# leohuang2013/pyannote-audio_speaker-diarization_cpp

Hardware: AMD Instinct MI355X
Metric: real-time factor (audio-sec/wall-sec), 1 h 16 kHz mono per GPU (higher is better)
Workload: dtype f32

## Files before the change

pyannote-audio_speaker-diarization_cpp_amd/csrc/api.cpp:

```cpp
#include "common.h"
#include <algorithm>
#include <cmath>
#include <cstdlib>

static std::string g_create_err;

int seg_prec(const sd_ctx* c) { return c->seg_precision >= 0 ? c->seg_precision : (c->ecapa_precision != 0 ? 3 : 0); }

extern "C" const char* sd_create_error(void) { return g_create_err.c_str(); }
extern "C" const char* sd_last_error(const sd_ctx* c) { return c ? c->err.c_str() : "null context"; }

extern "C" sd_ctx* sd_create(const char* seg_path, const char* emb_path, int device)
{
    g_create_err.clear();
    int ndev = 0;
    if (hipGetDeviceCount(&ndev) != hipSuccess || ndev <= 0) { g_create_err = "no HIP device available (libsdhip has no CPU fallback)"; return nullptr; }
    if (device < 0 || device >= ndev) { g_create_err = "device id out of range"; return nullptr; }
    if (hipSetDevice(device) != hipSuccess) { g_create_err = "hipSetDevice failed"; return nullptr; }
    sd_ctx* c = new sd_ctx();
    c->device = device;
    hipDeviceProp_t prop;
    if (hipGetDeviceProperties(&prop, device) == hipSuccess) c->num_cu = prop.multiProcessorCount;
    if (hipStreamCreateWithFlags(&c->stream, hipStreamNonBlocking) != hipSuccess) { g_create_err = "hipStreamCreate failed"; delete c; return nullptr; }
    auto fail = [&](const std::string& m) { g_create_err = m; sd_destroy(c); return (sd_ctx*)nullptr; };
// ... 28 lines not shown
    while (!c->streams.empty()) sd_stream_close(c->streams.back());
    for (void* p : c->owned) (void)hipFree(p);
    for (auto& kv : c->ws) kv.second.release();
    if (c->stream) (void)hipStreamDestroy(c->stream);
    delete c;
}

void sd_flush_profile(sd_ctx* c)
{
    for (auto& t : c->pending) {
        hipEvent_t e0 = std::get<1>(t), e1 = std::get<2>(t);
        float ms = 0;
        if (hipEventSynchronize(e1) == hipSuccess) (void)hipEventElapsedTime(&ms, e0, e1);
        KernelStat& s = c->stats[std::get<0>(t)];
        s.ms += ms; s.launches++; s.flops += std::get<3>(t); s.bytes += std::get<4>(t);
        (void)hipEventDestroy(e0); (void)hipEventDestroy(e1);
    }
    c->pending.clear();
}

extern "C" int sd_kernel_stats(const sd_ctx* cc, const char* kernel, double* total_ms, int64_t* launches, double* flops, double* bytes)
{
    sd_ctx* c = const_cast<sd_ctx*>(cc);
    if (!c || !kernel) return SD_ERR_ARG;
    (void)hipStreamSynchronize(c->stream);
    sd_flush_profile(c);
    auto it = c->stats.find(kernel);
    KernelStat s; if (it != c->stats.end()) s = it->second;
    if (total_ms) *total_ms = s.ms; if (launches) *launches = s.launches; if (flops) *flops = s.flops; if (bytes) *bytes = s.bytes;
    return SD_OK;
}
extern "C" int sd_debug_read_ws(sd_ctx* c, const char* name, int64_t offset, void* h_out, int64_t bytes)
{
    if (!c || !name || !h_out || offset < 0 || bytes < 0) return SD_ERR_ARG;
    auto it = c->ws.find(name);
    if (it == c->ws.end() || !it->second.p) SD_FAIL(c, SD_ERR_ARG, "no workspace named %s", name);
    if ((size_t)(offset + bytes) > it->second.cap) SD_FAIL(c, SD_ERR_ARG, "workspace %s holds %zu bytes", name, it->second.cap);
    HIPCHK(c, hipStreamSynchronize(c->stream));
    HIPCHK(c, hipMemcpy(h_out, (const char*)it->second.p + offset, (size_t)bytes, hipMemcpyDeviceToHost));
    return SD_OK;
}
extern "C" void sd_reset_stats(sd_ctx* c) { if (!c) return; (void)hipStreamSynchronize(c->stream); sd_flush_profile(c); c->stats.clear(); }
extern "C" int sd_stage_ms(const sd_ctx* c, double* ms4) { if (!c || !ms4) return SD_ERR_ARG; for (int i = 0; i < 4; ++i) ms4[i] = c->stage_ms[i]; return SD_OK; }
extern "C" int sd_set_option(sd_ctx* c, const char* key, int64_t v)
{
    if (!c || !key) return SD_ERR_ARG;
    std::string k(key);
    if (k == "emb_batch_items") { c->emb_batch_items = v; c->emb_batch_explicit = true; }
    else if (k == "seg_batch_chunks") c->seg_batch_chunks = v;
    else if (k == "ws_limit_mb") g_ws_limit.store(v > 0 ? (size_t)v << 20 : 0);
    else if (k == "emb_batch_default") { c->emb_batch_items = 3072; c->emb_batch_explicit = false; c->embed_calls = v; }
    else if (k == "linkage_wgs") c->linkage_wgs = v;
    else if (k == "linkage_threads") c->linkage_threads = v;
    else if (k == "linkage_kernel") c->linkage_kernel = v;
    else if (k == "linkage_tie_kernel") c->linkage_tie_kernel = v;
    else if (k == "linkage_zero_phase") c->linkage_zero_phase = v;
    else if (k == "linkage_force_heap") c->linkage_force_heap = v != 0;
    else if (k == "linkage_hx_wide") c->linkage_hx_wide = v != 0;
    else if (k == "linkage_prefetch") c->linkage_prefetch = v != 0;
    else if (k == "linkage_one_xcd") c->linkage_one_xcd = v;
    else if (k == "linkage_square") c->linkage_square = v;
    else if (k == "skip_dead_rows") c->skip_dead_rows = v != 0;
    else if (k == "conv_h256") c->conv_h256 = v != 0;
    else if (k == "conv_glds") c->conv_glds = v != 0;
    else if (k == "conv_pp") c->conv_pp = v != 0;
    else if (k == "conv_glds_f32") c->conv_glds_f32 = v != 0;
    else if (k == "conv_mfma16") { if (v < 0 || v > 2) return SD_ERR_ARG; c->conv_mfma16 = (int)v; }
    else if (k == "conv_rot") { if (v < 0 || v > 3) return SD_ERR_ARG; c->conv_rot = (int)v; }
    else if (k == "conv_stagger") { if (v < 0 || v > 2) return SD_ERR_ARG; c->conv_stagger = (int)v; }
    else if (k == "conv_w256_f32") c->conv_w256_f32 = v != 0;
    else if (k == "conv_pn") c->conv_pn = (int)v;
    else if (k == "ecapa_ld_pad") { if (v < 0 || v > 1024 || ((int64_t)v & 7)) return SD_ERR_ARG; c->ecapa_ld_pad = (int)v; }
    else if (k == "seg_shared_conv0") c->seg_shared_conv0 = v != 0;
    else if (k == "seg_wide_ih") c->seg_wide_ih = v != 0;
    else if (k == "conv_w256_kmin") c->conv_w256_kmin = (int)v;
    else if (k == "conv_pn128") c->conv_pn128 = (int)v;
    else if (k == "seg_precision") { if (v != 0 && v != 3 && v != -1) SD_FAIL(c, SD_ERR_ARG, "seg_precision must be 0 (f32), 3 (split fp16 operands for the LSTM) or -1 (auto: 3 whenever ecapa_precision is not 0)"); c->seg_precision = (int)v; }
    else if (k == "ecapa_precision") { if (v < 0 || v > 3) SD_FAIL(c, SD_ERR_ARG, "ecapa_precision must be 0 (f32), 1 (fp16), 2 (fp16, hi + lo weight planes) or 3 (f32 tensors, split fp16 operands on the wide layers)");
                                        if (hipSetDevice(c->device) != hipSuccess) SD_FAIL(c, SD_ERR_HIP, "hipSetDevice failed");
                                        const int rcw = ensure_ecapa_mode_weights(c, (int)v); if (rcw) return rcw;
                                        c->ecapa_precision = (int)v; }
    else if (k == "ecapa_f16_hp") { if (v != 0 && v != 1 && v != 3) SD_FAIL(c, SD_ERR_ARG, "ecapa_f16_hp must be 0, 1 (MFA output in f32) or 3 (+ the attention branch)"); c->ecapa_f16_hp = (int)v; }
    else if (k == "ecapa_keep_cat") c->ecapa_keep_cat = v != 0;
    else if (k == "rank0_permille") c->rank0_permille = (int)v;
    else if (k == "virtual_world") c->virtual_world = (int)v;
    else if (k == "comm_timeout_ms") c->comm_timeout_ms = v;
    else if (k == "inject_fail_rank") c->inject_fail_rank = (int)v;
    else if (k == "constrained_assignment") c->constrained_assignment = v != 0;
    else if (k == "clustering_method") { if (v < SD_LINKAGE_SINGLE || v > SD_LINKAGE_WEIGHTED) SD_FAIL(c, SD_ERR_ARG, "clustering_method must be one of SD_LINKAGE_SINGLE (0) .. SD_LINKAGE_WEIGHTED (6)"); c->clustering_method = (int)v; }
    else if (k == "min_cluster_size") { if (v < 1 || v > 0x7fffffff) SD_FAIL(c, SD_ERR_ARG, "min_cluster_size must be at least 1"); c->min_cluster_size = (int)v; }
    else if (k == "num_clusters") c->num_clusters = (int)v;
    else if (k == "min_clusters") c->min_clusters = (int)v;
    else if (k == "max_clusters") c->max_clusters = (int)v;
    else if (k == "activity_hamming") { if (v != 0 && v != 1) SD_FAIL(c, SD_ERR_ARG, "activity_hamming must be 0 or 1"); c->activity_hamming = v != 0; }
    else if (k == "profile") { c->profile = v != 0; c->profile_detail = v >= 2; }
    else SD_FAIL(c, SD_ERR_ARG, "unknown option %s", key);
    return SD_OK;
}

extern "C" int sd_set_option_f64(sd_ctx* c, const char* key, double v)
{
    if (!c || !key) return SD_ERR_ARG;
    std::string k(key);
    if (k == "clustering_threshold") { if (!(v >= 0.0 && v <= 2.0)) SD_FAIL(c, SD_ERR_ARG, "clustering_threshold must lie in [0, 2]"); c->clustering_threshold = v; }
    else if (k == "activity_onset") { if (!(v >= 0.0 && v <= 1.0)) SD_FAIL(c, SD_ERR_ARG, "activity_onset must lie in [0, 1]"); c->activity_onset = v; }
    else if (k == "activity_offset") { if (!(v >= 0.0 && v <= 1.0)) SD_FAIL(c, SD_ERR_ARG, "activity_offset must lie in [0, 1]"); c->activity_offset = v; }
    else if (k == "activity_min_duration_on") { if (!(v >= 0.0)) SD_FAIL(c, SD_ERR_ARG, "activity_min_duration_on must be >= 0"); c->activity_min_on = v; }
    else if (k == "activity_min_duration_off") { if (!(v >= 0.0)) SD_FAIL(c, SD_ERR_ARG, "activity_min_duration_off must be >= 0"); c->activity_min_off = v; }
    else SD_FAIL(c, SD_ERR_ARG, "unknown real-valued option %s", key);
    return SD_OK;
}
extern "C" int sd_linkage_method_from_name(const char* name)
{
    static const char* const names[] = {"single", "complete", "average", "centroid", "median", "ward", "weighted"};
    if (!name) return -1;
    for (int i = 0; i < 7; ++i) if (std::string(name) == names[i]) return i;
    return -1;
}

extern "C" int64_t sd_num_chunks(int64_t n, int64_t* last_len)
{
    int64_t i = 0, cnt = 0;
    if (n > SD_CHUNK) { cnt = (n - SD_CHUNK + SD_HOP - 1) / SD_HOP; i = cnt * SD_HOP; }
    int64_t ll = 0;
    if (i + 1 < n) { ll = n - i; cnt++; }
    if (last_len) *last_len = ll;
    return cnt;
}

extern "C" int sd_embed_dev(sd_ctx* c, const float* d_wav, int64_t n, const float* d_masks, int64_t items, int64_t first_item, float* d_emb)
{
    ENTER(c);
    if (!d_wav || !d_masks || !d_emb || n <= 0 || items < 0) SD_FAIL(c, SD_ERR_ARG, "sd_embed_dev: bad argument");
    int rc = run_embed(c, d_wav, n, d_masks, items, first_item, d_emb);
    if (rc) return rc;
    HIPCHK(c, hipStreamSynchronize(c->stream));
    return SD_OK;
}

extern "C" int sd_embed(sd_ctx* c, const float* h_wav, int64_t n, const float* h_masks, int64_t items, float* h_emb)
{
    ENTER(c);
    if (!h_wav || !h_masks || !h_emb || n <= 0 || items < 0) SD_FAIL(c, SD_ERR_ARG, "sd_embed: bad argument");
    DTMP(c, dw, n * sizeof(float)); DTMP(c, dm, items * SD_FRAMES * sizeof(float)); DTMP(c, de, items * SD_EMB_DIM * sizeof(float));
    HIPCHK(c, hipMemcpy(dw.p, h_wav, n * sizeof(float), hipMemcpyHostToDevice));
    HIPCHK(c, hipMemcpy(dm.p, h_masks, items * SD_FRAMES * sizeof(float), hipMemcpyHostToDevice));
    int rc = run_embed(c, (const float*)dw.p, n, (const float*)dm.p, items, 0, (float*)de.p);
    if (rc) return rc;
    HIPCHK(c, hipStreamSynchronize(c->stream));
    HIPCHK(c, hipMemcpy(h_emb, de.p, items * SD_EMB_DIM * sizeof(float), hipMemcpyDeviceToHost));
    return SD_OK;
}

extern "C" int sd_frontend(sd_ctx* c, const float* h_wav, int64_t n, const float* h_masks, int64_t items, float* h_feats, float* h_lens)
{
    ENTER(c);
    if (!h_wav || !h_masks || n <= 0 || items <= 0) SD_FAIL(c, SD_ERR_ARG, "sd_frontend: bad argument");
    DTMP(c, dw, n * sizeof(float)); DTMP(c, dm, items * SD_FRAMES * sizeof(float));
    DTMP(c, df, items * SD_TP * SD_FEAT_LD * sizeof(float)); DTMP(c, dl, items * sizeof(float));
    DTMP(c, dn, items * sizeof(int)); DTMP(c, dv, items * sizeof(int)); DTMP(c, dg, items * sizeof(int)); DTMP(c, dr, (items + 1) * sizeof(int));
    HIPCHK(c, hipMemcpy(dw.p, h_wav, n * sizeof(float), hipMemcpyHostToDevice));
    HIPCHK(c, hipMemcpy(dm.p, h_masks, items * SD_FRAMES * sizeof(float), hipMemcpyHostToDevice));
    std::vector<int> ro((size_t)items + 1);
    for (int64_t i = 0; i <= items; ++i) ro[(size_t)i] = (int)(i * SD_TP);
    HIPCHK(c, hipMemcpy(dr.p, ro.data(), ro.size() * sizeof(int), hipMemcpyHostToDevice));
    int rc = frontend_prepare(c, (const float*)dm.p, items, 0, (float*)dl.p, (int*)dn.p, (int*)dv.p, (int*)dg.p, false, nullptr, nullptr);
// ... 238 lines not shown
```

pyannote-audio_speaker-diarization_cpp_amd/csrc/common.h:

```cpp
#pragma once
#include <hip/hip_runtime.h>
#include <atomic>
#include <chrono>
#include <cstdint>
#include <cstdio>
#include <cstring>
#include <map>
#include <set>
#include <string>
#include <functional>
#include <initializer_list>
#include <vector>
#include "../../include/sdhip_test.h"

#define SD_T 501
#define SD_TP 501
#define SD_NBINS 201
#define SD_NMELS 80
#define SD_FEAT_LD 96

struct KernelStat { double ms = 0; int64_t launches = 0; double flops = 0, bytes = 0; };

inline std::atomic<long long> g_ws_alloc_us{0}, g_ws_free_us{0};
inline std::atomic<size_t> g_ws_alloc_bytes{0}, g_ws_allocs{0};
// ... 42 lines not shown
    int TpIn, TpOut;
    int Tin, T;
    int Cin, Cout, KT, dil;
    int cin_real;
    int pad_mode;
    int act1, act2;
    int m_tiles, n_tiles;
    int sched;
    const int2* rowtab;
    int in_rows;
    int y_f32;
    int kt_real;
    int prec;
    const void* W16x;
    float acc_scale;
    int stagger;
};
#define ROWTAB_T(y) ((y) & 1023)
#define ROWTAB_LAST(y) (((y) >> 10) & 1023)
#define ROWTAB_ITEM(y) ((int)((unsigned)(y) >> 20))
#define ROWTAB_MAX_ITEMS 4095
#define SD_SKINNY_MAX_ROWS 4096

struct EcapaWeights {
    bool loaded = false;
    float* mel_w = nullptr; int* mel_lo = nullptr; int* mel_cnt = nullptr; int* mel_off = nullptr; int mel_nnz = 0;
    float* window = nullptr;
    double* tw_cos = nullptr;
    double* tw_nsin = nullptr;
    ConvLayer block0;
    struct SERes { ConvLayer tdnn1, res[7], tdnn2, se1, se2; int dil; } blk[3];
    ConvLayer mfa, asp_tdnn_x, asp_tdnn_ms, asp_conv, fc;
    int C = 1024;
    std::vector<ConvLayer*> conv16;
    bool have16 = false, have16x = false;
};

struct SegWeights {
    bool loaded = false;
    float wn_w = 1, wn_b = 0;
    ConvLayer conv0, conv1, conv2;
    float* conv0_wsum = nullptr;
    float* in_w[3] = {nullptr, nullptr, nullptr};
    float* in_b[3] = {nullptr, nullptr, nullptr};
    ConvLayer lstm_ih[4];
    float* lstm_hh[4][2] = {};
    void* lstm_hh_x[4][2] = {};
    float lstm_hh_inv[4][2] = {};
    ConvLayer lin0, lin1;
    float* cls_w = nullptr; float* cls_b = nullptr;
};

struct StepStash {
    bool clustered = false;
    int64_t N = 0; int K = 0;
    std::vector<int> clusters, cluster_res, hard_pre;
    std::vector<double> X, Xn, soft;
    int64_t ar0 = 0, cr0 = 0, rows = 0, crow_all = 0, nact = 0;
    int64_t infer_items = 0;
};

struct sd_ctx {
    int device = 0;
    hipStream_t stream = nullptr;
    std::string err;
    EcapaWeights ew;
    SegWeights sw;
    std::vector<void*> owned;
    char* warena_cur = nullptr; size_t warena_left = 0;
    std::map<std::string, DevBuf> ws;
    std::set<std::string> rs_taps_filled;
    std::map<std::string, KernelStat> stats;
    bool profile = false;
    bool profile_detail = false;
    std::vector<std::tuple<std::string, hipEvent_t, hipEvent_t, double, double>> pending;
    double stage_ms[4] = {0, 0, 0, 0};
    int64_t emb_batch_items = 3072;
    bool emb_batch_explicit = false;
    int64_t embed_calls = 0;
    int64_t seg_batch_chunks = 4096;
    int num_clusters = -1, min_clusters = -1, max_clusters = -1;
    int ecapa_precision = 0;
    int seg_precision = -1;
    bool ecapa_keep_cat = false;
    int ecapa_f16_hp = 0;
    bool conv_w256_f32 = true;
    int conv_pn128 = 0;
    int ecapa_ld_pad = 0;
    bool wav_padded = false;
    bool seg_wide_ih = true;
    bool seg_shared_conv0 = true;
    int conv_w256_kmin = 0;
    int conv_pn = 0;
    bool conv_h256 = true;
    int conv_mfma16 = 1;
    int conv_rot = 3;
    int conv_stagger = 0;
    bool conv_glds_f32 = false;
    bool conv_pp = true;
    bool conv_glds = true;
    bool skip_dead_rows = true;
    int64_t linkage_wgs = -1;
    int64_t linkage_square = -1;
    int64_t linkage_one_xcd = 1;
    int64_t linkage_zero_phase = 1;
    int64_t linkage_tie_kernel = 1;
    int64_t linkage_prefetch = 0;
    bool linkage_hx_wide = false;
    bool linkage_force_heap = false;
    int64_t linkage_kernel = -1;
    int64_t linkage_threads = 0;
    int num_cu = 256;
    bool constrained_assignment = false;
    int clustering_method = SD_LINKAGE_CENTROID;
    double clustering_threshold = (double)0.7153814381597874f;
    int min_cluster_size = 15;
    std::vector<double> last_conf;
    double activity_onset = 0.5, activity_offset = 0.5, activity_min_on = 0.0, activity_min_off = 0.0;
    bool activity_hamming = false;
    std::vector<double> last_activity;
    int64_t fe_bill_samples = -1, fe_bill_frames = 0;
    int64_t wav_origin = 0;
    void* comm = nullptr;
    int rank = 0, world = 1;
    int virtual_world = 0;
    int64_t comm_timeout_ms = 600000;
    int64_t job_seq = 0;
    int inject_fail_rank = -1;
    int rank0_permille = -1;
    std::string dump_dir;
    int dump_level = 0;
    StepStash stash;
    std::string ws_failed;
    const char* last_conv_kernel = nullptr;
    const float* planted_scores = nullptr;
    const float* planted_emb = nullptr;
    int64_t planted_lo = 0, planted_n = 0;
    std::vector<sd_stream*> streams;
};

#define SD_FAIL(ctx, code, ...) do { char _b[512]; snprintf(_b, sizeof(_b), __VA_ARGS__); (ctx)->err = _b; return (code); } while (0)
#define HIPCHK(ctx, expr) do { hipError_t _e = (expr); if (_e != hipSuccess) { SD_FAIL(ctx, SD_ERR_HIP, "%s failed: %s (%s:%d)", #expr, hipGetErrorString(_e), __FILE__, __LINE__); } } while (0)
#define KCHECK(ctx) HIPCHK(ctx, hipGetLastError())

template <class T> inline T* ws_get(sd_ctx* c, const char* name, size_t count) {
    DevBuf& b = c->ws[name];
    if (b.reserve(count * sizeof(T))) { c->ws_failed = name; return nullptr; }
    return b.as<T>();
}
#define WS(ctx, T, var, name, count) T* var = ws_get<T>(ctx, name, (size_t)(count)); if (!var) SD_FAIL(ctx, SD_ERR_HIP, "hipMalloc of workspace %s (%zu bytes) failed", name, (size_t)(count) * sizeof(T))

struct DevTmp {
    void* p = nullptr;
    ~DevTmp() { if (p) (void)hipFree(p); }
    int alloc(size_t bytes) { return hipMalloc(&p, bytes ? bytes : 16) == hipSuccess ? 0 : 1; }
};
#define DTMP(ctx, var, bytes) DevTmp var; if (var.alloc(bytes)) SD_FAIL(ctx, SD_ERR_HIP, "hipMalloc(%zu) failed", (size_t)(bytes))
#define ENTER(ctx) do { if (!(ctx)) return SD_ERR_ARG; (ctx)->err.clear(); if (hipSetDevice((ctx)->device) != hipSuccess) SD_FAIL(ctx, SD_ERR_HIP, "hipSetDevice failed"); } while (0)
#define GRID1(n) dim3((unsigned)(((n) + 255) / 256)), dim3(256)
inline double now_ms() { return std::chrono::duration<double, std::milli>(std::chrono::steady_clock::now().time_since_epoch()).count(); }

struct ProfScope {
    sd_ctx* c; std::string name; hipEvent_t e0 = nullptr, e1 = nullptr; double flops, bytes;
    ProfScope(sd_ctx* ctx, const std::string& n, double fl = 0, double by = 0) : c(ctx), name(n), flops(fl), bytes(by) {
        if (c->profile) { (void)hipEventCreate(&e0); (void)hipEventCreate(&e1); (void)hipEventRecord(e0, c->stream); }
    }
    ~ProfScope() {
        if (c->profile) { (void)hipEventRecord(e1, c->stream); c->pending.emplace_back(name, e0, e1, flops, bytes); }
        else { KernelStat& s = c->stats[name]; s.launches++; s.flops += flops; s.bytes += bytes; }
    }
};
void sd_flush_profile(sd_ctx* c);

inline int conv_tiles_grid(const sd_ctx* c, ConvArgs& a, int tile_m, int tile_n, int wgs_per_cu)
{
    a.m_tiles = (a.M + tile_m - 1) / tile_m;
    a.n_tiles = (a.Cout + tile_n - 1) / tile_n;
    int g = (wgs_per_cu * c->num_cu / 8) * 8;
    if (g < 8) g = 8;
    const int lx_max = ((a.m_tiles + 7) / 8) * a.n_tiles;
    if (g / 8 > lx_max) g = lx_max * 8;
    return g;
}
struct ConvBill { double flops, bytes; };
inline ConvBill conv_bill(const ConvArgs& a, double rows, bool f16, int inputs = 1)
{
    const int cin = a.cin_real > 0 ? a.cin_real : a.Cin;
    const int kt_alg = a.kt_real > 0 ? a.kt_real : a.KT;
    return {2.0 * rows * a.Cout * cin * kt_alg, (f16 ? 2.0 : 4.0) * (rows * cin * inputs + rows * a.Cout + (double)a.Cout * cin * a.KT)};
}
inline bool conv_set_dyn_lds(const sd_ctx* c, std::atomic<unsigned>& mask, std::initializer_list<const void*> kernels, size_t lds_bytes)
{
    const unsigned dev_bit = 1u << (c->device & 31);
    if (mask.load(std::memory_order_acquire) & dev_bit) return true;
    for (const void* k : kernels)
        if (hipFuncSetAttribute(k, hipFuncAttributeMaxDynamicSharedMemorySize, (int)lds_bytes) != hipSuccess) { (void)hipGetLastError(); return false; }
    mask.fetch_or(dev_bit, std::memory_order_release);
    return true;
}
struct ConvProfWide {
    ProfScope all, prec, wide, caller;
    ConvProfWide(sd_ctx* c, const char* tag, const char* p, const ConvBill& b)
        : all(c, c->profile_detail ? std::string("conv_gemm:") + tag : std::string("conv_gemm"), b.flops, b.bytes),
          prec(c, std::string("conv_gemm_") + p, b.flops, b.bytes), wide(c, std::string("conv_w256_") + p, b.flops, b.bytes),
          caller(c, strcmp(tag, "lstm_ih") == 0 ? "conv_w256_seg" : "conv_w256_ecapa", b.flops, b.bytes) {}
};
int launch_conv_gemm(sd_ctx* c, const ConvArgs& a, const char* tag);
int launch_conv_gemm_h256(sd_ctx* c, const ConvArgs& a, const char* tag);
int launch_conv_gemm_g256(sd_ctx* c, const ConvArgs& a, const char* tag);
int launch_conv_gemm_pp(sd_ctx* c, const ConvArgs& a, const char* tag);
int seg_prec(const sd_ctx* c);
int launch_conv_narrow(sd_ctx* c, const ConvArgs& a, const char* tag);
struct PackTensor { std::vector<int64_t> dims; std::vector<float> data; };
typedef std::map<std::string, PackTensor> Pack;
int load_pack(const char* path, Pack& out, std::string& err);
int load_model_any(const char* path, int kind, Pack& out, std::string& err);
int build_ecapa_weights(sd_ctx* c, const Pack& p);
int build_seg_weights(sd_ctx* c, const Pack& p);
float lstm_whh_split(const float* whh , _Float16* planes );
void* weight_alloc(sd_ctx* c, size_t bytes);
int ensure_ecapa_mode_weights(sd_ctx* c, int ecapa_precision);
inline size_t conv_w16_bytes(const ConvLayer& L) { return (size_t)2 * L.KT * L.Cout * L.CinPad16 * 2; }
inline size_t conv_w16x_bytes(const ConvLayer& L) { return (size_t)2 * L.KT * L.Cout * L.CinPad * 2; }
int build_conv_w16(sd_ctx* c, ConvLayer& L, void* d);
int build_conv_w16x(sd_ctx* c, ConvLayer& L, void* d, unsigned* d_max);
int frontend_prepare(sd_ctx* c, const float* d_masks, int64_t items, int64_t first_item, float* d_wav_lens, int* d_nnorm, int* d_nvalid,
                     int* d_flags, bool compact, int* h_n_active, int* d_cidx, std::vector<int>* h_nvalid = nullptr);
int frontend_features(sd_ctx* c, const float* d_wav, int64_t n, int64_t first_item, int64_t run_items, bool compact, const int* d_nnorm,
                      const int* d_rowoff, float* d_feats , bool sig_mode = false);
int frontend_prepare_signals(sd_ctx* c, int64_t items);
#define EC_SPACES 4
struct EcapaRowPlan {
    int64_t n = 0;
    std::vector<int> off[EC_SPACES];
    const int* d_off = nullptr;
};
int ecapa_need_rows(int nvalid, bool skip_dead_rows);
int ecapa_build_rowtab(sd_ctx* c, const int* d_off_out, int base_out, const int* d_off_in, int base_in, int64_t items, int2* d_rowtab);
int ecapa_rows_to_half(sd_ctx* c, const float* d_f32, void* d_f16, int64_t n4);
int ecapa_row_plan(sd_ctx* c, const int* h_nvalid, int64_t n, EcapaRowPlan& plan, int* d_off );
int run_ecapa(sd_ctx* c, const float* d_feats, const int* d_nvalid , const EcapaRowPlan& plan, int64_t a0, int64_t a1, float* d_emb );
std::vector<int64_t> ecapa_plan_batches(const EcapaRowPlan& plan, int64_t cap_rows, bool balance);
int64_t ecapa_round_items(int64_t nb);
int ecapa_run_items(sd_ctx* c, const float* d_feats, const int* d_nvalid, const EcapaRowPlan& plan, int64_t nb, bool balance, float* d_emb);
int run_embed(sd_ctx* c, const float* d_wav, int64_t n, const float* d_masks, int64_t items, int64_t first_item, float* d_emb);
int run_segment(sd_ctx* c, const float* d_wav, int64_t n, int64_t chunk_lo, int64_t chunk_hi, float* d_seg);
int run_segment_rows(sd_ctx* c, const float* d_rows, int64_t rows, int T, float* d_seg, int* frames);
int launch_chunk_norm(sd_ctx* c, const float* d_wav, int64_t origin, int64_t first_chunk, int64_t hop, int L, int64_t chunks, float w, float b, float* xn);
int launch_chunk_stats(sd_ctx* c, const float* d_wav, int64_t origin, int64_t first_chunk, int L, int64_t chunks, float w, float b, float2* st);
int launch_pool_norm(sd_ctx* c, int stage, const float* in, int64_t chunks, int Lc, const float* gw, const float* gb, float* out,
                     const float2* cst, const float* wsum, int chunk_rows);
int launch_lstm_rec(sd_ctx* c, const float* G, const float* whh_f, const float* whh_b, const void* whx_f, const void* whx_b, float inv_f, float inv_b,
                    float* H, int64_t B, int F);
int launch_classifier(sd_ctx* c, const float* y, const float* W, const float* bias, float* seg, int64_t chunks, int F);
int run_postseg(sd_ctx* c, const float* d_seg, int64_t chunks, uint8_t* d_bin, float* d_masks, int* d_nact);
int run_count(sd_ctx* c, const uint8_t* d_bin, int64_t chunks, int32_t* d_count, int64_t n_count, double* d_avg = nullptr);
int write_step_dumps(sd_ctx* c, const float* d_seg, const float* d_emb, int64_t chunks, int64_t n_samples, const std::vector<int>& hard_post, int K);
int64_t count_frames_host(int64_t chunks);
int sd_np_rint_host(double v);
int64_t closest_frame_host(double w_start, double w_step, double w_dur, double t);
int run_linkage(sd_ctx* c, const double* d_X, int64_t N, int d, double* d_Z, int method = SD_LINKAGE_CENTROID, int metric = SD_METRIC_EUCLIDEAN);
int run_cluster_labels(sd_ctx* c, const double* d_X, int64_t N, int d, double cutoff, std::vector<int>& labels1, std::vector<double>* Zout = nullptr,
                       int method = SD_LINKAGE_CENTROID, int metric = SD_METRIC_EUCLIDEAN);
int run_clustering(sd_ctx* c, const double* d_emb , int64_t M, int d, std::vector<int>& hard, int* K,
                   int num_clusters = -1, int min_clusters = -1, int max_clusters = -1, std::vector<double>* soft_best = nullptr);
void fcluster_host(const std::vector<double>& Z, int64_t n, double cutoff, std::vector<int>& T);
int64_t activity_frames_host(int64_t chunks);
int64_t activity_rows_host(int64_t nf, int64_t n_samples);
int run_activity_scores(sd_ctx* c, const float* d_seg, int64_t chunks, int kind, double* d_scores, int64_t nf);
int run_activity_regions(sd_ctx* c, const double* d_scores, int64_t rows, int label, std::vector<sd_turn>& turns);
int run_reconstruct(sd_ctx* c, const float* d_seg, const int* d_nact, const int* d_hard, const int32_t* d_count,
                    int64_t n_count, int64_t chunks, int64_t n_samples, int K, std::vector<sd_turn>& turns);
```

pyannote-audio_speaker-diarization_cpp_amd/csrc/ecapa.hip:

```cpp
#include "common.h"
#include <algorithm>

template <class T> __global__ void k_masked_mean(const T* __restrict__ x, int ld, const int* __restrict__ nvalid, const int* __restrict__ rowoff, int row_base,
                              float* __restrict__ out, int C)
{
    const int item = blockIdx.y, ch = blockIdx.x * blockDim.x + threadIdx.x;
    if (ch >= C) return;
    const int nv = nvalid[item];
    const T* p = x + (size_t)(rowoff[item] - row_base) * ld + ch;
    float s0 = 0, s1 = 0, s2 = 0, s3 = 0;
    int t = 0;
    for (; t + 3 < nv; t += 4) { s0 += (float)p[(size_t)t * ld]; s1 += (float)p[(size_t)(t + 1) * ld]; s2 += (float)p[(size_t)(t + 2) * ld]; s3 += (float)p[(size_t)(t + 3) * ld]; }
    for (; t < nv; ++t) s0 += (float)p[(size_t)t * ld];
    out[(size_t)item * C + ch] = ((s0 + s1) + (s2 + s3)) / (float)nv;
}

template <class T> struct Vec4;
template <> struct Vec4<float> { typedef float4 type; };
template <> struct Vec4<_Float16> { typedef _Float16 type __attribute__((ext_vector_type(4))); };
template <class T> __device__ __forceinline__ float4 ld4(const T* p)
{
    if constexpr (sizeof(T) == 4) return *(const float4*)p;
    else { const typename Vec4<_Float16>::type h = *(const typename Vec4<_Float16>::type*)p; return make_float4((float)h[0], (float)h[1], (float)h[2], (float)h[3]); }
}
// ... 175 lines not shown
    WS(c, T, mfa, "ec_mfa", MN * LD3);
    WS(c, T, hid, "ec_hid", MN * 128);
    WS(c, float, se_s, "ec_se_s", items * C);
    WS(c, float, se_h, "ec_se_h", items * 128);
    WS(c, float, se_g, "ec_se_g", items * C);
    WS(c, float, ms, "ec_ms", items * 2 * C3);
    WS(c, float, ib, "ec_ib", items * 128);
    WS(c, float, pooled, "ec_pooled", items * 2 * C3);
    int rc;
    hipStream_t st = c->stream;
    int2* tabs[EC_SPACES][EC_SPACES] = {};
    auto tab = [&](int so, int si) -> int2* {
        if (tabs[so][si]) return tabs[so][si];
        char key[32]; snprintf(key, sizeof(key), "ec_rowtab_%d%d", so, si);
        int2* p = ws_get<int2>(c, key, (size_t)R[so] + 128);
        if (!p) return nullptr;
        if (ecapa_build_rowtab(c, ro[so], rbase[so], ro[si], rbase[si], items, p)) return nullptr;
        tabs[so][si] = p;
        return p;
    };
#define TAB(var, so, si) int2* var = tab(so, si); if (!var) SD_FAIL(c, SD_ERR_HIP, "hipMalloc of a row table failed")

    const void* f_in = d_feats; int f_ld = SD_FEAT_LD;
    if (sizeof(T) == 2) {
        WS(c, _Float16, fh, "ec_feats16", M * 128);
        hipLaunchKernelGGL(k_feats_to_half, GRID1(M * 128), 0, st, d_feats, fh, M);
        KCHECK(c);
        f_in = fh; f_ld = 128;
    }
    { TAB(t00, 0, 0); ConvArgs a = conv_args(E.block0, f_in, f_ld, x0, LD, M, true, P); a.act1 = 1; a.rowtab = t00; if ((rc = launch_conv_gemm(c, a, "block0"))) return rc; }

    for (int b = 0; b < 3; ++b) {
        const auto& B = E.blk[b];
        const int cs = b, os = b + 1, is = b == 0 ? 0 : 1;
        const int64_t Mc = R[cs], Mo = R[os];
        const T* xin = (b == 0) ? x0 : cat + (size_t)(b - 1) * C;
        const int xin_ld = (b == 0) ? LD : LD3;
        TAB(t_in, cs, is); TAB(t_cc, cs, cs); TAB(t_oc, os, cs);
        { ConvArgs a = conv_args(B.tdnn1, xin, xin_ld, tr, LDT, Mc, true, P); a.act1 = 1; a.rowtab = t_in; a.in_rows = (int)R[is]; if ((rc = launch_conv_gemm(c, a, "tdnn1"))) return rc; }
        const int S = C / 8;
        for (int i = 1; i < 8; ++i) {
            ConvArgs a = conv_args(B.res[i - 1], tr + (i - 1) * S, LDT, tr + C + (i - 1) * S, LDT, Mc, true, P);
            a.act1 = 1;
            if (i >= 2) { a.X2 = (const float*)(tr + C + (i - 2) * S); a.x2_ld = LDT; }
            a.rowtab = t_cc;
            if ((rc = launch_conv_gemm(c, a, "res2net"))) return rc;
        }
        { ConvArgs a = conv_args(B.tdnn2, tr + C - S, LDT, t2, LD, Mo, true, P); a.act1 = 1; a.rowtab = t_oc; a.in_rows = (int)Mc; if ((rc = launch_conv_gemm(c, a, "tdnn2"))) return rc; }
        {
            ProfScope ps(c, "se_mean", 0, (double)Mo * C * 4.0);
            hipLaunchKernelGGL(k_masked_mean<T>, dim3((C + 255) / 256, (unsigned)items), dim3(256), 0, st, t2, LD, d_nvalid, ro[os], rbase[os], se_s, C);
            KCHECK(c);
        }
        { ConvArgs a = conv_args(B.se1, se_s, C, se_h, 128, items, false); a.act1 = 1; if ((rc = launch_conv_gemm(c, a, "se1"))) return rc; }
        { ConvArgs a = conv_args(B.se2, se_h, 128, se_g, C, items, false); a.act2 = 2; if ((rc = launch_conv_gemm(c, a, "se2"))) return rc; }
        {
            const int2* res_map = nullptr; const int2* out_map = nullptr;
            if (os != is) { TAB(m, os, is); res_map = m; }
            if (os != 1) { TAB(m, os, 1); out_map = m; }
            ProfScope ps(c, "se_apply", 0, (double)Mo * C * 12.0);
            hipLaunchKernelGGL(k_se_apply<T>, GRID1(Mo * (C / 4)), 0, st, t2, LD, se_g, xin, xin_ld, cat + (size_t)b * C, LD3, C, Mo, t_oc, res_map, out_map);
            KCHECK(c);
        }
    }
    TAB(t31, 3, 1); TAB(t33, 3, 3);
    const int hp = sizeof(T) == 2 ? c->ecapa_f16_hp : 0;
    float* mfa32 = nullptr;
    if (hp & 1) { WS(c, float, m32, "ec_mfa32", MN * LD3); mfa32 = m32; }
    {
        ConvArgs a = conv_args(E.mfa, cat, LD3, mfa32 ? (void*)mfa32 : (void*)mfa, LD3, MN, true, P);
        a.act1 = 1; a.rowtab = t31; a.in_rows = (int)R[1]; a.y_f32 = mfa32 ? 1 : 0;
        if ((rc = launch_conv_gemm(c, a, "mfa"))) return rc;
    }
    if (mfa32 && !(hp & 2)) {
        if ((rc = ecapa_rows_to_half(c, mfa32, mfa, MN * LD3 / 4))) return rc;
    }
    {
        ProfScope ps(c, "asp_stats", 0, (double)MN * C3 * 4.0);
        if (mfa32) hipLaunchKernelGGL(k_asp_stats<float>, dim3((C3 + 255) / 256, (unsigned)items), dim3(256), 0, st, mfa32, LD3, d_nvalid, ro[3], rbase[3], ms, C3);
        else hipLaunchKernelGGL(k_asp_stats<T>, dim3((C3 + 255) / 256, (unsigned)items), dim3(256), 0, st, mfa, LD3, d_nvalid, ro[3], rbase[3], ms, C3);
        KCHECK(c);
    }
    { ConvArgs a = conv_args(E.asp_tdnn_ms, ms, 2 * C3, ib, 128, items, false); if ((rc = launch_conv_gemm(c, a, "asp_ms"))) return rc; }
    float* logits;
    if (sizeof(T) == 2 || c->ecapa_keep_cat) { WS(c, float, lg, "ec_logits", MN * LD3); logits = lg; } else logits = (float*)cat;
    if (hp & 2) {
        WS(c, float, hid32, "ec_hid32", MN * 128);
        { ConvArgs a = conv_args(E.asp_tdnn_x, mfa32, LD3, hid32, 128, MN, true, 0); a.act1 = 1; a.act2 = 1; a.item_bias = ib; a.ib_ld = 128; a.rowtab = t33; if ((rc = launch_conv_gemm(c, a, "asp_tdnn"))) return rc; }
        { ConvArgs a = conv_args(E.asp_conv, hid32, 128, logits, LD3, MN, true, 0); a.rowtab = t33; if ((rc = launch_conv_gemm(c, a, "asp_conv"))) return rc; }
    } else {
        { ConvArgs a = conv_args(E.asp_tdnn_x, mfa, LD3, hid, 128, MN, true, P); a.act1 = 1; a.act2 = 1; a.item_bias = ib; a.ib_ld = 128; a.rowtab = t33; if ((rc = launch_conv_gemm(c, a, "asp_tdnn"))) return rc; }
        { ConvArgs a = conv_args(E.asp_conv, hid, 128, logits, LD3, MN, true, P); a.rowtab = t33; a.y_f32 = 1; if ((rc = launch_conv_gemm(c, a, "asp_conv"))) return rc; }
    }
    {
        ProfScope ps(c, "asp_pool", 0, (double)MN * C3 * 8.0);
        if (mfa32) hipLaunchKernelGGL(k_asp_pool<float>, dim3((C3 + 255) / 256, (unsigned)items), dim3(256), 0, st, mfa32, logits, LD3, d_nvalid, ro[3], rbase[3], pooled, C3);
        else hipLaunchKernelGGL(k_asp_pool<T>, dim3((C3 + 255) / 256, (unsigned)items), dim3(256), 0, st, mfa, logits, LD3, d_nvalid, ro[3], rbase[3], pooled, C3);
        KCHECK(c);
    }
    { ConvArgs a = conv_args(E.fc, pooled, 2 * C3, d_emb, SD_EMB_DIM, items, false); if ((rc = launch_conv_gemm(c, a, "fc"))) return rc; }
    return SD_OK;
}

__global__ void k_flag_nonfinite(const float* e, int64_t n, int* flag)
{
    const int64_t i = (int64_t)blockIdx.x * blockDim.x + threadIdx.x;
    if (i < n && !isfinite(e[i])) *flag = 1;
}

int run_ecapa(sd_ctx* c, const float* d_feats, const int* d_nvalid, const EcapaRowPlan& plan, int64_t a0, int64_t a1, float* d_emb)
{
    if (c->ecapa_precision == 1 || c->ecapa_precision == 2) return run_ecapa_t<_Float16>(c, d_feats, d_nvalid, plan, a0, a1, d_emb);
    const int rc = run_ecapa_t<float>(c, d_feats, d_nvalid, plan, a0, a1, d_emb);
    if (rc == SD_OK && c->ecapa_precision == 3 && a1 > a0) {
        WS(c, int, flag, "ec_x3_flag", 1);
        hipLaunchKernelGGL(k_flag_nonfinite, GRID1((a1 - a0) * SD_EMB_DIM), 0, c->stream, d_emb + (size_t)a0 * SD_EMB_DIM, (a1 - a0) * SD_EMB_DIM, flag);
        KCHECK(c);
    }
    return rc;
}

static int ecapa_run_batches(sd_ctx* c, const std::function<int()>& batches)
{
    if (c->ecapa_precision != 3) return batches();
    WS(c, int, flag, "ec_x3_flag", 1);
    HIPCHK(c, hipMemsetAsync(flag, 0, sizeof(int), c->stream));
    int rc = batches();
    if (rc) return rc;
    int h = 0;
    HIPCHK(c, hipMemcpyAsync(&h, flag, sizeof(int), hipMemcpyDeviceToHost, c->stream));
    HIPCHK(c, hipStreamSynchronize(c->stream));
    if (!h) return SD_OK;
    c->stats["x3_overflow_fallbacks"].launches += 1;
    c->ecapa_precision = 0;
    rc = batches();
    c->ecapa_precision = 3;
    return rc;
}

static int64_t ec_fill_offsets(const int* h_nvalid, int64_t n, bool skip_dead_rows, EcapaRowPlan& plan)
{
    plan.n = n;
    for (int sp = 0; sp < EC_SPACES; ++sp) {
        std::vector<int>& off = plan.off[sp];
        off.assign((size_t)n + 1, 0);
        int64_t acc = 0;
        for (int64_t i = 0; i < n; ++i) { off[(size_t)i] = (int)acc; acc += ec_space_rows(h_nvalid[i], skip_dead_rows, sp); }
        if (acc > 0x7fffffff / 4) return acc;
        off[(size_t)n] = (int)acc;
    }
    return 0;
}
int ecapa_row_plan(sd_ctx* c, const int* h_nvalid, int64_t n, EcapaRowPlan& plan, int* d_off)
{
    plan.d_off = d_off;
    if (const int64_t over = ec_fill_offsets(h_nvalid, n, c->skip_dead_rows, plan))
        SD_FAIL(c, SD_ERR_ARG, "embedding stage: %lld feature rows in one shard (limit %d)", (long long)over, 0x7fffffff / 4);
    for (int sp = 0; sp < EC_SPACES; ++sp)
        HIPCHK(c, hipMemcpyAsync(d_off + (size_t)sp * (n + 1), plan.off[sp].data(), (size_t)(n + 1) * sizeof(int), hipMemcpyHostToDevice, c->stream));
    HIPCHK(c, hipStreamSynchronize(c->stream));
    return SD_OK;
}

int64_t ecapa_round_items(int64_t nb) { nb = (nb / 96) * 96; return nb < 96 ? 96 : nb; }

std::vector<int64_t> ecapa_plan_batches(const EcapaRowPlan& plan, int64_t cap_rows, bool balance)
{
    const std::vector<int>& rowoff = plan.off[0];
    const int64_t n = plan.n, rows_all = rowoff[(size_t)n];
    auto batch_efficiency = [&](int64_t a0, int64_t a1) -> double {
        static const int L[9][2] = {{0, 400}, {0, 1024}, {1, 1024}, {1, 1024}, {2, 1024}, {2, 1024}, {3, 1024}, {3, 3 * 3072}, {3, 2 * 128}};
        double ideal = 0.0, actual = 0.0;
        for (int l = 0; l < 9; ++l) {
            const int64_t M = plan.off[L[l][0]][(size_t)a1] - plan.off[L[l][0]][(size_t)a0];
            ideal += (double)L[l][1] * (double)M / 16384.0;
            actual += (double)L[l][1] * (double)((M + 16383) / 16384);
        }
// ... 112 lines not shown
```

Before: 2950.

## Fuse ECAPA attentive-pooling conv with softmax statistics pooling in one MFMA kernel

Adds a kernel that computes the ASP 128->C3 pointwise conv with f32 MFMA from LDS-staged hidden rows and immediately folds the logits into an online softmax-weighted mean and variance per channel. Items are partitioned across persistent slots sized to the CU count. The change avoids writing and re-reading the MN x C3 logits tensor and drops one launch. It applies only to the f32 path without row padding, and adds a more complex kernel with double buffering and a Welford-style merge whose numerics differ slightly from the two-pass version.

```diff
diff --git a/pyannote-audio_speaker-diarization_cpp_amd/csrc/api.cpp b/pyannote-audio_speaker-diarization_cpp_amd/csrc/api.cpp
--- a/pyannote-audio_speaker-diarization_cpp_amd/csrc/api.cpp
+++ b/pyannote-audio_speaker-diarization_cpp_amd/csrc/api.cpp
@@ -134,6 +134,7 @@
                                         c->ecapa_precision = (int)v; }
     else if (k == "ecapa_f16_hp") { if (v != 0 && v != 1 && v != 3) SD_FAIL(c, SD_ERR_ARG, "ecapa_f16_hp must be 0, 1 (MFA output in f32) or 3 (+ the attention branch)"); c->ecapa_f16_hp = (int)v; }
     else if (k == "ecapa_keep_cat") c->ecapa_keep_cat = v != 0;
+    else if (k == "ecapa_asp_fused") c->ecapa_asp_fused = v != 0;
     else if (k == "rank0_permille") c->rank0_permille = (int)v;
     else if (k == "virtual_world") c->virtual_world = (int)v;
     else if (k == "comm_timeout_ms") c->comm_timeout_ms = v;
diff --git a/pyannote-audio_speaker-diarization_cpp_amd/csrc/asp_fused.hip b/pyannote-audio_speaker-diarization_cpp_amd/csrc/asp_fused.hip
--- /dev/null
+++ b/pyannote-audio_speaker-diarization_cpp_amd/csrc/asp_fused.hip
@@ -0,0 +1,173 @@
+#include "common.h"
+#include <memory>
+
+typedef float f32x16 __attribute__((ext_vector_type(16)));
+
+#define ASPF_WAVES 8
+#define ASPF_COLS (32 * ASPF_WAVES)
+#define ASPF_CBG 4
+#define ASPF_K 128
+#define ASPF_HLD 132
+
+__global__ __launch_bounds__(64 * ASPF_WAVES)
+void k_asp_conv_pool(const float* __restrict__ hid, const float* __restrict__ x, int ld, const float* __restrict__ Wt, const float* __restrict__ bias,
+                     const float* __restrict__ scale, const float* __restrict__ shift, const int* __restrict__ nvalid, const int* __restrict__ rowoff,
+                     int row_base, float* __restrict__ pooled, int C3, int items, int slots, int MN)
+{
+    const int id = blockIdx.x;
+    const int grp = (id / (8 * ASPF_CBG)) * 8 + (id & 7), cb = (id >> 3) % ASPF_CBG;
+    const int gps = C3 / (ASPF_COLS * ASPF_CBG);
+    const int slot = grp / gps;
+    if (slot >= slots) return;
+    const int lane = threadIdx.x & 63, wv = threadIdx.x >> 6, li = lane & 31, lh = lane >> 5;
+    const int ch = ((grp - slot * gps) * ASPF_CBG + cb) * ASPF_COLS + wv * 32 + li;
+
+    auto first_item = [&](int64_t target) {
+        int lo = 0, hi = items;
+        while (lo < hi) { const int mid = (lo + hi) >> 1; if ((int64_t)(rowoff[mid] - row_base) < target) lo = mid + 1; else hi = mid; }
+        return lo;
+    };
+    const int it0 = first_item(((int64_t)MN * slot + slots - 1) / slots), it1 = first_item(((int64_t)MN * (slot + 1) + slots - 1) / slots);
+    if (it0 >= it1) return;
+
+    __shared__ __attribute__((aligned(16))) float hbuf[2][32 * ASPF_HLD];
+    float wr[64];
+    {
+        const float* wrow = Wt + (size_t)ch * ASPF_K + 64 * lh;
+#pragma unroll
+        for (int s = 0; s < 64; s += 4) {
+            const float4 v = *(const float4*)(wrow + s);
+            wr[s] = v.x; wr[s + 1] = v.y; wr[s + 2] = v.z; wr[s + 3] = v.w;
+        }
+    }
+    const float cbias = bias ? bias[ch] : 0.0f, cs = scale ? scale[ch] : 1.0f, csh = scale ? shift[ch] : 0.0f;
+    const float c1 = cs * 1.44269504f, c2 = (cbias * cs + csh) * 1.44269504f;
+
+    int item = it0, t0 = 0, nv = nvalid[it0];
+    int64_t r0 = rowoff[it0] - row_base;
+    bool have = true;
+    int p_item = 0, p_t0 = 0, p_nv = 0;
+    bool p_last = false;
+    const int sr = threadIdx.x >> 5, sc = (threadIdx.x & 31) * 4;
+    {
+        const float4 g0 = *(const float4*)(hid + (r0 + min(sr, nv - 1)) * ASPF_K + sc);
+        const float4 g1 = *(const float4*)(hid + (r0 + min(sr + 16, nv - 1)) * ASPF_K + sc);
+        *(float4*)&hbuf[0][sr * ASPF_HLD + sc] = g0;
+        *(float4*)&hbuf[0][(sr + 16) * ASPF_HLD + sc] = g1;
+    }
+    float xq[16];
+    f32x16 accq;
+#pragma unroll
+    for (int r = 0; r < 16; ++r) { xq[r] = 0.0f; accq[r] = 0.0f; }
+    float mx = -INFINITY, W = 0.0f, mean = 0.0f, m2 = 0.0f;
+    int cur = 0;
+    __syncthreads();
+
+#pragma unroll 2
+    for (;;) {
+        const bool last = t0 + 32 >= nv;
+        int n_item = item, n_t0 = t0 + 32, n_nv = nv;
+        int64_t n_r0 = r0;
+        bool n_have = have;
+        if (last) {
+            n_t0 = 0;
+            if (have && item + 1 < it1) { n_item = item + 1; n_nv = nvalid[n_item]; n_r0 = rowoff[n_item] - row_base; }
+            else n_have = false;
+        }
+        const float* xp = x + r0 * ld + ch;
+        const float4 g0 = *(const float4*)(hid + (n_r0 + min(n_t0 + sr, n_nv - 1)) * ASPF_K + sc);
+        const float4 g1 = *(const float4*)(hid + (n_r0 + min(n_t0 + sr + 16, n_nv - 1)) * ASPF_K + sc);
+        float xv[16];
+#pragma unroll
+        for (int r = 0; r < 16; ++r) xv[r] = xp[(int64_t)min(t0 + (r & 3) + 8 * (r >> 2) + 4 * lh, nv - 1) * ld];
+        __builtin_amdgcn_sched_barrier(0);
+        f32x16 acc;
+#pragma unroll
+        for (int r = 0; r < 16; ++r) acc[r] = 0.0f;
+        const float* hb = &hbuf[cur][li * ASPF_HLD + lh * 64];
+#pragma unroll
+        for (int s = 0; s < 64; s += 4) {
+            const float4 a = *(const float4*)(hb + s);
+            acc = __builtin_amdgcn_mfma_f32_32x32x2f32(a.x, wr[s], acc, 0, 0, 0);
+            acc = __builtin_amdgcn_mfma_f32_32x32x2f32(a.y, wr[s + 1], acc, 0, 0, 0);
+            acc = __builtin_amdgcn_mfma_f32_32x32x2f32(a.z, wr[s + 2], acc, 0, 0, 0);
+            acc = __builtin_amdgcn_mfma_f32_32x32x2f32(a.w, wr[s + 3], acc, 0, 0, 0);
+        }
+        float lg[16], mb = -INFINITY;
+#pragma unroll
+        for (int r = 0; r < 16; ++r) {
+            const bool ok = p_t0 + (r & 3) + 8 * (r >> 2) + 4 * lh < p_nv;
+            lg[r] = ok ? fmaf(accq[r], c1, c2) : -INFINITY;
+            mb = fmaxf(mb, lg[r]);
+        }
+        const float mn = fmaxf(mx, mb);
+        const float s = __builtin_amdgcn_exp2f(mx - mn);
+        float Wb = 0.0f, Sx = 0.0f;
+#pragma unroll
+        for (int r = 0; r < 16; ++r) {
+            lg[r] = __builtin_amdgcn_exp2f(lg[r] - mn);
+            Wb += lg[r];
+            Sx = fmaf(lg[r], xq[r], Sx);
+        }
+        const float mean_b = Sx * __builtin_amdgcn_rcpf(Wb);
+        float m2b = 0.0f;
+#pragma unroll
+        for (int r = 0; r < 16; ++r) { const float d = xq[r] - mean_b; m2b = fmaf(lg[r] * d, d, m2b); }
+        {
+            const float Wa = W * s, Wn = Wa + Wb, dl = mean_b - mean, rn = __builtin_amdgcn_rcpf(Wn);
+            const float mean_n = fmaf(dl, Wb * rn, mean), m2n = fmaf(m2, s, m2b) + dl * dl * (Wa * Wb * rn);
+            const bool any = mb > -INFINITY;
+            mx = any ? mn : mx; W = any ? Wn : W; mean = any ? mean_n : mean; m2 = any ? m2n : m2;
+        }
+        if (p_last) {
+            const float mxb = __shfl_down(mx, 32), Wb = __shfl_down(W, 32), meanb = __shfl_down(mean, 32), m2b = __shfl_down(m2, 32);
+            if (lh == 0) {
+                if (Wb > 0.0f) {
+                    if (W > 0.0f) {
+                        const float m = fmaxf(mx, mxb);
+                        const float sa = __builtin_amdgcn_exp2f(mx - m), sb = __builtin_amdgcn_exp2f(mxb - m);
+                        const float wa = W * sa, wb = Wb * sb, d = meanb - mean;
+                        W = wa + wb;
+                        mean = mean + d * wb / W;
+                        m2 = m2 * sa + m2b * sb + d * d * wa * wb / W;
+                    } else { W = Wb; mean = meanb; m2 = m2b; }
+                }
+                pooled[(size_t)p_item * 2 * C3 + ch] = mean;
+                pooled[(size_t)p_item * 2 * C3 + C3 + ch] = sqrtf(fmaxf(m2 / W, 1e-12f));
+            }
+            mx = -INFINITY; W = 0.0f; mean = 0.0f; m2 = 0.0f;
+        }
+        if (!have) break;
+        *(float4*)&hbuf[cur ^ 1][sr * ASPF_HLD + sc] = g0;
+        *(float4*)&hbuf[cur ^ 1][(sr + 16) * ASPF_HLD + sc] = g1;
+        __syncthreads();
+        cur ^= 1;
+        p_item = item; p_t0 = t0; p_nv = nv; p_last = last;
+        accq = acc;
+#pragma unroll
+        for (int r = 0; r < 16; ++r) xq[r] = xv[r];
+        item = n_item; t0 = n_t0; nv = n_nv; r0 = n_r0; have = n_have;
+    }
+}
+
+bool asp_fused_fits(const ConvLayer& L, int C3) { return L.Cin == ASPF_K && L.CinPad == ASPF_K && L.KT == 1 && L.Cout == C3 && C3 % (ASPF_COLS * ASPF_CBG) == 0; }
+
+int launch_asp_conv_pool(sd_ctx* c, const float* hid, const float* x, int ld, const ConvLayer& L, const int* d_nvalid, const int* d_rowoff, int row_base,
+                         float* pooled, int C3, int64_t items, int64_t MN)
+{
+    if (!asp_fused_fits(L, C3)) SD_FAIL(c, SD_ERR_ARG, "asp_conv_pool: layer %d -> %d (k%d) does not fit the kernel", L.Cin, L.Cout, L.KT);
+    const int gps = C3 / (ASPF_COLS * ASPF_CBG);
+    int64_t slots = (c->num_cu / ASPF_CBG) / gps;
+    if (slots > items) slots = items;
+    if (slots < 1) slots = 1;
+    const int groups = (int)slots * gps;
+    const unsigned grid = (unsigned)(((groups + 7) / 8) * 8 * ASPF_CBG);
+    const double flops = 2.0 * (double)MN * ASPF_K * C3, bytes = (double)MN * (C3 + ASPF_K) * 4.0;
+    ProfScope ps(c, "asp_pool", flops, bytes);
+    std::unique_ptr<ProfScope> pd;
+    if (c->profile_detail) pd.reset(new ProfScope(c, "asp_conv_pool", flops, bytes));
+    hipLaunchKernelGGL(k_asp_conv_pool, dim3(grid), dim3(64 * ASPF_WAVES), 0, c->stream, hid, x, ld, L.W, L.bias, L.scale, L.shift, d_nvalid, d_rowoff,
+                       row_base, pooled, C3, (int)items, (int)slots, (int)MN);
+    KCHECK(c);
+    return SD_OK;
+}
diff --git a/pyannote-audio_speaker-diarization_cpp_amd/csrc/common.h b/pyannote-audio_speaker-diarization_cpp_amd/csrc/common.h
--- a/pyannote-audio_speaker-diarization_cpp_amd/csrc/common.h
+++ b/pyannote-audio_speaker-diarization_cpp_amd/csrc/common.h
@@ -148,6 +148,7 @@
     int num_clusters = -1, min_clusters = -1, max_clusters = -1;
     int ecapa_precision = 0;
     int seg_precision = -1;
+    bool ecapa_asp_fused = true;
     bool ecapa_keep_cat = false;
     int ecapa_f16_hp = 0;
     bool conv_w256_f32 = true;
@@ -310,6 +311,9 @@
 int64_t ecapa_round_items(int64_t nb);
 int ecapa_run_items(sd_ctx* c, const float* d_feats, const int* d_nvalid, const EcapaRowPlan& plan, int64_t nb, bool balance, float* d_emb);
 int run_embed(sd_ctx* c, const float* d_wav, int64_t n, const float* d_masks, int64_t items, int64_t first_item, float* d_emb);
+bool asp_fused_fits(const ConvLayer& asp_conv, int C3);
+int launch_asp_conv_pool(sd_ctx* c, const float* hid , const float* x , int ld, const ConvLayer& asp_conv, const int* d_nvalid,
+                         const int* d_rowoff , int row_base, float* pooled, int C3, int64_t items, int64_t MN);
 int run_segment(sd_ctx* c, const float* d_wav, int64_t n, int64_t chunk_lo, int64_t chunk_hi, float* d_seg);
 int run_segment_rows(sd_ctx* c, const float* d_rows, int64_t rows, int T, float* d_seg, int* frames);
 int launch_chunk_norm(sd_ctx* c, const float* d_wav, int64_t origin, int64_t first_chunk, int64_t hop, int L, int64_t chunks, float w, float b, float* xn);
diff --git a/pyannote-audio_speaker-diarization_cpp_amd/csrc/ecapa.hip b/pyannote-audio_speaker-diarization_cpp_amd/csrc/ecapa.hip
--- a/pyannote-audio_speaker-diarization_cpp_amd/csrc/ecapa.hip
+++ b/pyannote-audio_speaker-diarization_cpp_amd/csrc/ecapa.hip
@@ -281,9 +281,14 @@
         KCHECK(c);
     }
     { ConvArgs a = conv_args(E.asp_tdnn_ms, ms, 2 * C3, ib, 128, items, false); if ((rc = launch_conv_gemm(c, a, "asp_ms"))) return rc; }
-    float* logits;
-    if (sizeof(T) == 2 || c->ecapa_keep_cat) { WS(c, float, lg, "ec_logits", MN * LD3); logits = lg; } else logits = (float*)cat;
-    if (hp & 2) {
+    const bool fused = sizeof(T) == 4 && P == 0 && c->ecapa_asp_fused && asp_fused_fits(E.asp_conv, C3);
+    float* logits = nullptr;
+    if (!fused) { if (sizeof(T) == 2 || c->ecapa_keep_cat) { WS(c, float, lg, "ec_logits", MN * LD3); logits = lg; } else logits = (float*)cat; }
+    if (fused) {
+        { ConvArgs a = conv_args(E.asp_tdnn_x, mfa, LD3, hid, 128, MN, true, P); a.act1 = 1; a.act2 = 1; a.item_bias = ib; a.ib_ld = 128; a.rowtab = t33; if ((rc = launch_conv_gemm(c, a, "asp_tdnn"))) return rc; }
+        if ((rc = launch_asp_conv_pool(c, (const float*)(const void*)hid, (const float*)(const void*)mfa, LD3, E.asp_conv, d_nvalid, ro[3], rbase[3], pooled, C3, items, MN))) return rc;
+    }
+    else if (hp & 2) {
         WS(c, float, hid32, "ec_hid32", MN * 128);
         { ConvArgs a = conv_args(E.asp_tdnn_x, mfa32, LD3, hid32, 128, MN, true, 0); a.act1 = 1; a.act2 = 1; a.item_bias = ib; a.ib_ld = 128; a.rowtab = t33; if ((rc = launch_conv_gemm(c, a, "asp_tdnn"))) return rc; }
         { ConvArgs a = conv_args(E.asp_conv, hid32, 128, logits, LD3, MN, true, 0); a.rowtab = t33; if ((rc = launch_conv_gemm(c, a, "asp_conv"))) return rc; }
@@ -291,7 +296,7 @@
         { ConvArgs a = conv_args(E.asp_tdnn_x, mfa, LD3, hid, 128, MN, true, P); a.act1 = 1; a.act2 = 1; a.item_bias = ib; a.ib_ld = 128; a.rowtab = t33; if ((rc = launch_conv_gemm(c, a, "asp_tdnn"))) return rc; }
         { ConvArgs a = conv_args(E.asp_conv, hid, 128, logits, LD3, MN, true, P); a.rowtab = t33; a.y_f32 = 1; if ((rc = launch_conv_gemm(c, a, "asp_conv"))) return rc; }
     }
-    {
+    if (!fused) {
         ProfScope ps(c, "asp_pool", 0, (double)MN * C3 * 8.0);
         if (mfa32) hipLaunchKernelGGL(k_asp_pool<float>, dim3((C3 + 255) / 256, (unsigned)items), dim3(256), 0, st, mfa32, logits, LD3, d_nvalid, ro[3], rbase[3], pooled, C3);
         else hipLaunchKernelGGL(k_asp_pool<T>, dim3((C3 + 255) / 256, (unsigned)items), dim3(256), 0, st, mfa, logits, LD3, d_nvalid, ro[3], rbase[3], pooled, C3);
```

Measured after the change: 2978, median of 6. No clear change (+0.9%).
